# Annusha/LIReC

Hardware: AMD Instinct MI355X
Metric: clips/sec fwd+bwd at 16 tracks×2048-d (higher is better)
Workload: dtype f32 in/out, bf16x3 split-precision MFMA, f32 accumulate

## Files before the change

### lirec_amd/csrc/gemm.hpp

```cpp
#pragma once
#include <hip/hip_runtime.h>
#include <stdint.h>

namespace lirec {

typedef float f32x16 __attribute__((ext_vector_type(16)));
typedef float f32x4 __attribute__((ext_vector_type(4)));

enum { L_NT = 0, L_NN = 1, L_TN = 2 };
enum { EPI_STORE = 0, EPI_DROP_RELU = 1, EPI_TANH_DROP = 2, EPI_RELU_BWD = 3, EPI_TANH_BWD = 4 };

struct GemmProblem {
  const float* A; const float* B; float* C;
  const float* bias;
  const float* rowscale;
  const float* aux;
  float* aux_out;
  float* dbias;
  long lda, ldb, ldc, ldaux;
  int M, N, K;
  int gs, gstride, goff;
  unsigned gs_magic;
  int epi; float beta;
  int dbias_set;
  unsigned seed_lo, seed_hi, site, thresh; float drop_scale; int drop_col_off;
  const unsigned long long* seed_dev;
  int x_bf16;
  int tiles_n, tile_start;
  int ksplit, kchunk, tiles_mn;
  float* slab; float* dbias_slab;
  const int* rowmap; const int* dyn;
  const int* srow;
  const void* A_lo; const void* B_lo;
  unsigned char* xq_out; long ld_xq;
};

struct AdamFuse {
  float* p; const float* g; float* m; float* v;
  float step_size, bc2_sqrt, beta1, beta2, eps, wd, gscale, lr;
  const long long* step_dev;
  int wq16c;
};
struct AdamHyperRow {
  float lr, beta1, beta2, eps, wd, decoupled, pad_[2];
// ... 33 lines not shown
    if constexpr (DECOUPLED) gg = gv[j] * ad.gscale;
    else gg = gv[j] * ad.gscale + ad.wd * pv[j];
    mv[j] = mv[j] + (1.f - ad.beta1) * (gg - mv[j]);
    vv[j] = vv[j] * ad.beta2 + (1.f - ad.beta2) * gg * gg;
    const float denom = sqrtf(vv[j]) / bc2_sqrt + ad.eps;
    if constexpr (DECOUPLED) pv[j] = pv[j] * decay;
    pv[j] = pv[j] - step_size * (mv[j] / denom);
  }
  *reinterpret_cast<f32x4*>(ad.p + off) = pv;
  *reinterpret_cast<f32x4*>(ad.m + off) = mv;
  *reinterpret_cast<f32x4*>(ad.v + off) = vv;
  return pv;
}

#define LIREC_MAX_PROB 8
struct GemmGroup {
  int nprob; int total_tiles; int ablate; int row_tiles;
  const int* nt_bound;
  int nt_bound_val;
  int p3_tm, p3_tn, p3_xm;
  int nt_ct_major;
  int onepass;
  int tier_rows, row_tiles2, first2;
  int pgroup;
  int tm_fast;
  int tiles_per_split, resident_slots, dyn_is_k;
  int dyn_split;
  float slab_cost, reduce_cost;
  GemmProblem p[LIREC_MAX_PROB];
};
struct GemmMeta { int site; int tag; };

inline bool gemm_problem_is_vec(int layout, const GemmProblem& p) {
  const bool a_kc = layout != 2, b_kc = layout == 0;
  const uintptr_t ma = (p.x_bf16 && layout == 0) ? 7 : 15, mb = (p.x_bf16 && layout == 2) ? 7 : 15;
  const bool va = ((p.lda & 3) == 0) && ((reinterpret_cast<uintptr_t>(p.A) & ma) == 0) && (((a_kc ? p.K : p.M) & 3) == 0);
  const bool vb = ((p.ldb & 3) == 0) && ((reinterpret_cast<uintptr_t>(p.B) & mb) == 0) && (((b_kc ? p.K : p.N) & 3) == 0);
  return va && vb;
}

__device__ __forceinline__ void philox4(unsigned c0, unsigned c1, unsigned c2, unsigned c3,
                                        unsigned k0, unsigned k1, unsigned out[4]) {
#pragma unroll 2
// ... 102 lines not shown
}

template <int ST = 64>
__device__ __forceinline__ int xcd_remap(int bid, int nwg) {
  const int full = nwg - nwg % (8 * ST);
  const int xcd = bid & 7;
  if (bid < full) {
    const int seq = bid >> 3;
    return ((seq / ST) * 8 + xcd) * ST + seq % ST;
  }
  const int n = nwg - full, q = n >> 3, r = n & 7;
  const int idx = (bid - full) >> 3;
  return full + (xcd < r ? xcd * (q + 1) : r * (q + 1) + (xcd - r) * q) + idx;
}

__device__ __forceinline__ int effective_ksplit(const GemmGroup& g, const GemmProblem& p, int K) {
  if (p.ksplit <= 1 || !g.dyn_split || !(g.ablate & 64)) return p.ksplit;
  int best = 1;
  float bestc = 3.0e38f;
  for (int ks = 1; ks <= p.ksplit; ++ks) {
    const int nk = ((K + ks - 1) / ks + 31) / 32;
    if (ks > 1 && nk < 8) break;
    const int rounds = (g.tiles_per_split * ks + g.resident_slots - 1) / g.resident_slots;
    const float c = (float)rounds * (float)nk + (ks > 1 ? g.reduce_cost + g.slab_cost * (float)(ks + 1) : 0.f);
    if (c < bestc) { bestc = c; best = ks; }
  }
  return best;
}

__device__ __forceinline__ int launch_tile(const GemmGroup& g) {
  int nwg = gridDim.x;
  if (g.dyn_split && g.dyn_is_k && (g.ablate & 64)) {
    const GemmProblem& p0 = g.p[0];
    const int ks = effective_ksplit(g, p0, dyn_limit(p0, p0.K));
    nwg = g.tiles_per_split * ks;
    if ((int)blockIdx.x >= nwg) return -1;
  }
  return g.pgroup > 0 ? xcd_remap<32>(blockIdx.x, nwg) : xcd_remap<64>(blockIdx.x, nwg);
}

struct TileCoord { int pi, split, m0, n0, tn, k_begin, k_end, M; };
template <int BM, int BN>
__device__ __forceinline__ TileCoord decode_tile(const GemmGroup& g, int tile, bool dyn_is_k) {
  TileCoord c;
  c.pi = 0;
  int tm;
  if (g.pgroup > 0) {
    const int G = g.pgroup, tier1 = g.tier_rows * g.row_tiles;
    const bool t2 = g.row_tiles2 > 0 && tile >= tier1;
    const int first = t2 ? g.first2 : 0, np = t2 ? g.nprob - g.first2 : g.nprob;
    const int rt = t2 ? g.row_tiles2 : g.row_tiles;
    const int rows = t2 ? g.p[first].tiles_mn / g.p[first].tiles_n - g.tier_rows : g.tier_rows;
    const int t = t2 ? tile - tier1 : tile;
    const int tn_each = g.p[first].tiles_n;
    const int blk = t / (G * rt);
    const int within = t - blk * G * rt;
    const int per = min(G, rows - blk * G) * tn_each;
    const int q = within / per, r2 = within - q * per;
    const int rot = (blk * np) / 8 + (t2 ? 1 : 0);
    c.pi = first + (q + rot) % np;
    const int pr = r2 / tn_each;
    c.tn = r2 - pr * tn_each;
    c.split = 0;
    tm = (t2 ? g.tier_rows : 0) + blk * G + pr;
  } else if (g.row_tiles > 0) {
    const int tier1 = g.tier_rows * g.row_tiles;
    if (g.row_tiles2 > 0 && tile >= tier1) {
      const int t2 = tile - tier1;
      const int row2 = t2 / g.row_tiles2;
      const int rem = t2 - row2 * g.row_tiles2 + g.p[g.first2].tile_start;
      c.pi = g.first2;
#pragma unroll
      for (int i = 1; i < LIREC_MAX_PROB; ++i)
        if (i > g.first2 && i < g.nprob && rem >= g.p[i].tile_start) c.pi = i;
      c.tn = rem - g.p[c.pi].tile_start;
      c.split = 0;
      tm = g.tier_rows + row2;
    } else {
      const int tiles_m = g.p[0].tiles_mn / g.p[0].tiles_n;
      int row, rem;
      if (g.tm_fast) {
        const int per_split = tiles_m * g.row_tiles;
        c.split = tile / per_split;
        const int r = tile - c.split * per_split;
        rem = r / tiles_m;
        tm = r - rem * tiles_m;
      } else {
        row = tile / g.row_tiles;
        rem = tile - row * g.row_tiles;
        c.split = row / tiles_m;
        tm = row - c.split * tiles_m;
      }
#pragma unroll
      for (int i = 1; i < LIREC_MAX_PROB; ++i)
        if (i < g.nprob && rem >= g.p[i].tile_start) c.pi = i;
      c.tn = rem - g.p[c.pi].tile_start;
    }
  } else {
#pragma unroll
    for (int i = 1; i < LIREC_MAX_PROB; ++i)
      if (i < g.nprob && tile >= g.p[i].tile_start) c.pi = i;
    int t = tile - g.p[c.pi].tile_start;
    c.split = t / g.p[c.pi].tiles_mn;
    t -= c.split * g.p[c.pi].tiles_mn;
    tm = t / g.p[c.pi].tiles_n;
    c.tn = t - tm * g.p[c.pi].tiles_n;
  }
  const GemmProblem& p = g.p[c.pi];
  c.m0 = tm * BM; c.n0 = c.tn * BN;
  int K = p.K, kchunk = p.kchunk;
  c.M = p.M;
  if (p.dyn) {
    if (dyn_is_k) {
      K = dyn_limit(p, p.K);
      const int ks = effective_ksplit(g, p, K);
      kchunk = ((K + ks - 1) / ks + 31) / 32 * 32;
      if (c.split >= ks) c.M = 0;
    } else {
      c.M = dyn_limit(p, p.M);
    }
  }
  c.k_begin = min(K, c.split * kchunk);
  c.k_end = min(K, c.k_begin + kchunk);
  return c;
}

template <int WM, int WN, int EPI>
__device__ __forceinline__ void gemm_epilogue_kind(const GemmProblem& p, const f32x16 (&acc)[WM][WN], int m0, int n0,
                                                   int wm0, int wn0, int lane, int M, bool have_rid = false, int rid_lane = 0) {
  constexpr bool USES_RND = (EPI == EPI_DROP_RELU || EPI == EPI_TANH_DROP || EPI == EPI_TANH_BWD);
  constexpr bool USES_AUX = (EPI == EPI_RELU_BWD || EPI == EPI_TANH_BWD);
  const int l31 = lane & 31, lh = lane >> 5;
  const int N = p.N;
  const bool drop = USES_RND && p.thresh != 0u;
  unsigned key_lo = p.seed_lo, key_hi = p.seed_hi;
  if (drop) apply_seed_offset(key_lo, key_hi, p.seed_dev);
  const bool mapped = drop && (p.rowmap != nullptr);
  const bool has_beta = p.beta != 0.f, has_rs = p.bias != nullptr && p.rowscale != nullptr;
  float bias_j[WN];
#pragma unroll
  for (int j = 0; j < WN; ++j) {
    const int col = n0 + wn0 + 32 * j + l31;
    bias_j[j] = (p.bias != nullptr && col < N) ? p.bias[col] : 0.f;
  }
  constexpr bool PRE_AUX = USES_AUX && (WM * WN <= 2);
#pragma unroll
  for (int i = 0; i < WM; ++i) {
#pragma unroll
    for (int j = 0; j < WN; ++j) {
      const int col = n0 + wn0 + 32 * j + l31;
      const bool colok = col < N;
      float axp[PRE_AUX ? 16 : 1];
      if constexpr (PRE_AUX) {
#pragma unroll
        for (int q = 0; q < 4; ++q)
#pragma unroll
          for (int jj = 0; jj < 4; ++jj) {
            const int row = m0 + wm0 + 32 * i + 8 * q + 4 * lh + jj;
            const bool okk = colok && row < M;
            axp[4 * q + jj] = p.aux[(long)(okk ? row : m0) * p.ldaux + (okk ? col : n0)];
          }
      }
#pragma unroll
      for (int q = 0; q < 4; ++q) {
        const int row4 = m0 + wm0 + 32 * i + 8 * q + 4 * lh;
        if (row4 >= M) continue;
        bool ok[4];
        float* cptr[4];
        float old[4] = {0.f, 0.f, 0.f, 0.f}, ax[4] = {0.f, 0.f, 0.f, 0.f}, rs[4] = {1.f, 1.f, 1.f, 1.f};
#pragma unroll
        for (int jj = 0; jj < 4; ++jj) {
          ok[jj] = colok && (row4 + jj < M);
          const int r = ok[jj] ? row4 + jj : m0, c = ok[jj] ? col : n0;
          cptr[jj] = p.C + (long)r * p.ldc + c;
          if (has_beta) old[jj] = *cptr[jj];
          if constexpr (PRE_AUX) ax[jj] = axp[4 * q + jj];
          else if constexpr (USES_AUX) ax[jj] = p.aux[(long)r * p.ldaux + c];
          if (has_rs) rs[jj] = p.rowscale[r];
        }
        unsigned w[4] = {0u, 0u, 0u, 0u};
        if (drop) {
          if (!mapped) {
            philox4((unsigned)(p.drop_col_off + col), (unsigned)(row4 >> 2), p.site, 0u, key_lo, key_hi, w);
          } else {
            unsigned rid[4], rnd[4];
#pragma unroll
            for (int jj = 0; jj < 4; ++jj) {
              if (have_rid) rid[jj] = (unsigned)__shfl(rid_lane, 32 * i + 8 * q + 4 * lh + jj, 64);
              else rid[jj] = (unsigned)p.rowmap[row4 + jj < M ? row4 + jj : M - 1];
            }
            unsigned blk = rid[0] >> 2;
            philox4((unsigned)(p.drop_col_off + col), blk, p.site, 0u, key_lo, key_hi, rnd);
#pragma unroll
// ... 26 lines not shown
          }
          if (ok[jj]) *cptr[jj] = v;
        }
        __asm__ volatile("" ::: "memory");
      }
    }
  }
}

__host__ __device__ constexpr bool epi_allowed(int layout, int epi) {
  return epi == EPI_STORE || (layout == L_NT && (epi == EPI_DROP_RELU || epi == EPI_TANH_DROP)) ||
         (layout == L_NN && (epi == EPI_RELU_BWD || epi == EPI_TANH_BWD));
}

template <int WM, int WN, int LAYOUT>
__device__ __forceinline__ void gemm_epilogue(const GemmProblem& p, const f32x16 (&acc)[WM][WN], int m0, int n0,
                                              int wm0, int wn0, int lane, int split, int M_eff, bool have_rid = false, int rid_lane = 0) {
  const int l31 = lane & 31, lh = lane >> 5;
  const int M = M_eff, N = p.N;
  if (p.ksplit > 1) {
    float* slab = p.slab + (long)split * p.M * N;
#pragma unroll
    for (int i = 0; i < WM; ++i)
#pragma unroll
      for (int j = 0; j < WN; ++j) {
        const int col = n0 + wn0 + 32 * j + l31;
#pragma unroll
        for (int r = 0; r < 16; ++r) {
          const int row = m0 + wm0 + 32 * i + (r & 3) + 8 * (r >> 2) + 4 * lh;
          if (row < M && col < N) slab[(long)row * N + col] = acc[i][j][r];
        }
      }
    return;
  }
  if constexpr (LAYOUT == L_NT) {
    if (p.epi == EPI_DROP_RELU) gemm_epilogue_kind<WM, WN, EPI_DROP_RELU>(p, acc, m0, n0, wm0, wn0, lane, M, have_rid, rid_lane);
    else if (p.epi == EPI_TANH_DROP) gemm_epilogue_kind<WM, WN, EPI_TANH_DROP>(p, acc, m0, n0, wm0, wn0, lane, M);
    else gemm_epilogue_kind<WM, WN, EPI_STORE>(p, acc, m0, n0, wm0, wn0, lane, M);
  } else if constexpr (LAYOUT == L_NN) {
    if (p.epi == EPI_RELU_BWD) gemm_epilogue_kind<WM, WN, EPI_RELU_BWD>(p, acc, m0, n0, wm0, wn0, lane, M);
    else if (p.epi == EPI_TANH_BWD) gemm_epilogue_kind<WM, WN, EPI_TANH_BWD>(p, acc, m0, n0, wm0, wn0, lane, M);
    else gemm_epilogue_kind<WM, WN, EPI_STORE>(p, acc, m0, n0, wm0, wn0, lane, M);
  } else {
    gemm_epilogue_kind<WM, WN, EPI_STORE>(p, acc, m0, n0, wm0, wn0, lane, M);
  }
}

static __global__ __launch_bounds__(256) void splitk_reduce_kernel(const GemmGroup g) {
  for (int pi = 0; pi < g.nprob; ++pi) {
    const GemmProblem& p = g.p[pi];
    if (p.ksplit <= 1) continue;
    const int ks = (p.dyn && g.dyn_is_k) ? effective_ksplit(g, p, dyn_limit(p, p.K)) : p.ksplit;
    const long mn = (long)p.M * p.N;
    const long gtid = (long)blockIdx.x * blockDim.x + threadIdx.x, gsz = (long)gridDim.x * blockDim.x;
    const bool vec4 = (p.N % 4 == 0) && (p.ldc % 4 == 0) && ((((size_t)p.C) | ((size_t)p.slab)) % 16 == 0);
    if (p.epi != EPI_STORE) {
      const bool drop = p.thresh != 0u && (p.epi == EPI_DROP_RELU || p.epi == EPI_TANH_DROP || p.epi == EPI_TANH_BWD);
      unsigned key_lo = p.seed_lo, key_hi = p.seed_hi;
      if (drop) apply_seed_offset(key_lo, key_hi, p.seed_dev);
      const long groups = (long)((p.M + 3) >> 2) * p.N;
      for (long e = gtid; e < groups; e += gsz) {
        const int r4 = (int)(e / p.N), col = (int)(e - (long)r4 * p.N), row0 = r4 << 2;
        float v[4] = {0.f, 0.f, 0.f, 0.f};
        for (int sidx = 0; sidx < ks; ++sidx) {
          const float* sl = p.slab + (long)sidx * mn + (long)row0 * p.N + col;
#pragma unroll
          for (int jj = 0; jj < 4; ++jj) if (row0 + jj < p.M) v[jj] += sl[(long)jj * p.N];
// ... 61 lines not shown
        *c = v;
      }
    }
    if (p.dbias && p.dbias_slab) {
      for (int m = blockIdx.x * blockDim.x + threadIdx.x; m < p.M; m += gridDim.x * blockDim.x) {
        float v = 0.f;
        for (int s = 0; s < ks; ++s) v += p.dbias_slab[(long)s * p.M + m];
        p.dbias[m] = p.dbias_set ? v : p.dbias[m] + v;
      }
    }
  }
}

struct ReducePlan { int n; int start[LIREC_MAX_PROB + 1]; int prob[LIREC_MAX_PROB]; };
static __global__ __launch_bounds__(256) void splitk_reduce_flat_kernel(const GemmGroup g, const ReducePlan rp) {
  int k = 0;
  while (k + 1 < rp.n && (int)blockIdx.x >= rp.start[k + 1]) ++k;
  const GemmProblem& p = g.p[rp.prob[k]];
  const int ks = p.ksplit;
  const long mn = (long)p.M * p.N;
  const long e = (long)((int)blockIdx.x - rp.start[k]) * 256 + threadIdx.x;
  const bool vec4 = (p.N % 4 == 0) && (p.ldc % 4 == 0) && ((((size_t)p.C) | ((size_t)p.slab)) % 16 == 0);
  if (vec4) {
    const long mn4 = mn >> 2;
    const int n4 = p.N >> 2;
    if (e < mn4) {
      const int row = (int)(e / n4), col = (int)(e - (long)row * n4) * 4;
      const f32x4* src = (const f32x4*)p.slab + e;
      f32x4* c = (f32x4*)(p.C + (long)row * p.ldc + col);
      f32x4 o = {0.f, 0.f, 0.f, 0.f};
      if (p.beta != 0.f) o = *c;
      f32x4 v = src[0];
      int s = 1;
      for (; s + 3 < ks; s += 4) {
        const f32x4 t0 = src[(long)s * mn4], t1 = src[(long)(s + 1) * mn4], t2 = src[(long)(s + 2) * mn4], t3 = src[(long)(s + 3) * mn4];
#pragma unroll
// ... 37 lines not shown

template <int LAYOUT, int WM, int WN, int TAG, bool VEC>
__global__ __launch_bounds__(256) void gemm_mfma_kernel(const GemmGroup g) {
  constexpr int BM = 64 * WM, BN = 64 * WN, BK = 32;
  constexpr bool A_KC = (LAYOUT != L_TN);
  constexpr bool B_KC = (LAYOUT == L_NT);
  constexpr int PA = A_KC ? BM + 1 : BM + 4;
  constexpr int PB = B_KC ? BN + 1 : BN + 4;
  constexpr int A_TILE = BK * PA, B_TILE = BK * PB;
  constexpr int CA = BM / 32, CB = BN / 32;
  __shared__ __attribute__((aligned(16))) float smem[2 * (A_TILE + B_TILE)];
  float* const As = smem;
  float* const Bs = smem + 2 * A_TILE;

  const int tid = threadIdx.x, lane = tid & 63, wave = tid >> 6;
  const int ltile = launch_tile(g);
  if (ltile < 0) return;
  const TileCoord tc = decode_tile<BM, BN>(g, ltile, LAYOUT == L_TN);
  const GemmProblem& p = g.p[tc.pi];
  const int m0 = tc.m0, n0 = tc.n0, tn = tc.tn;
  const int M = tc.M, N = p.N, K = tc.k_end;
  if (m0 >= M) return;

  const float* a_rowptr[CA];
  const float* b_rowptr[CB];
  bool a_rowok[CA], b_rowok[CB];
  if constexpr (A_KC) {
#pragma unroll
    for (int i = 0; i < CA; ++i) {
      const int m = m0 + (tid >> 3) + 32 * i;
      a_rowok[i] = m < M;
      a_rowptr[i] = p.A + (LAYOUT == L_NT ? phys_row(p, a_rowok[i] ? m : 0) : (long)(a_rowok[i] ? m : 0)) * p.lda;
    }
  }
  if constexpr (B_KC) {
#pragma unroll
    for (int i = 0; i < CB; ++i) {
// ... 120 lines not shown
    }
    if (do_dbias) {
      const float* ac = As + buf * A_TILE + tid;
      if (p.rowscale) {
        const int kbase = kb + kt * BK;
        for (int k = 0; k < BK; ++k) dbias_acc += ac[k * PA] * ((kbase + k < K) ? p.rowscale[kbase + k] : 0.f);
      } else {
#pragma unroll 8
        for (int k = 0; k < BK; ++k) dbias_acc += ac[k * PA];
      }
    }
    if (kt + 1 < nk) store_tiles(buf ^ 1, kb + (kt + 1) * BK);
    __syncthreads();
  }

  gemm_epilogue<WM, WN, LAYOUT>(p, acc, m0, n0, wm0, wn0, lane, tc.split, M);
  if (do_dbias && m0 + tid < M) {
    if (p.ksplit > 1) p.dbias_slab[(long)tc.split * p.M + m0 + tid] = dbias_acc;
    else p.dbias[m0 + tid] = p.dbias_set ? dbias_acc : p.dbias[m0 + tid] + dbias_acc;
  }
}

template <int LAYOUT>
__global__ void gemm_naive_kernel(const GemmProblem p) {
  const int col = blockIdx.x * 16 + (threadIdx.x & 15);
  const int row = blockIdx.y * 16 + (threadIdx.x >> 4);
  const int M = (LAYOUT == L_TN) ? p.M : dyn_limit(p, p.M);
  const int K = (LAYOUT == L_TN) ? dyn_limit(p, p.K) : p.K;
  if (row >= M || col >= p.N) return;
  float acc = 0.f;
  if (LAYOUT == L_NT) {
    const long arow = phys_row(p, row) * p.lda;
    const float* a = p.A + arow;
// ... 28 lines not shown
```

### lirec_amd/csrc/gemm_bf16x3.hpp

```cpp
#pragma once
#include <type_traits>
#include "gemm.hpp"

namespace lirec {

typedef __bf16 bf16x8 __attribute__((ext_vector_type(8)));
typedef __bf16 bf16x4 __attribute__((ext_vector_type(4)));
typedef short s16x4 __attribute__((ext_vector_type(4)));
typedef short s16x8 __attribute__((ext_vector_type(8)));

typedef float f32x2 __attribute__((ext_vector_type(2)));
typedef __bf16 bf16x2 __attribute__((ext_vector_type(2)));
__device__ __forceinline__ void split4(const f32x4 v, uint2& hi, uint2& lo) {
  const f32x2 v01 = {v[0], v[1]}, v23 = {v[2], v[3]};
  const bf16x2 h01 = __builtin_convertvector(v01, bf16x2), h23 = __builtin_convertvector(v23, bf16x2);
  const unsigned w01 = __builtin_bit_cast(unsigned, h01), w23 = __builtin_bit_cast(unsigned, h23);
  const f32x2 f01 = {__builtin_bit_cast(float, w01 << 16), __builtin_bit_cast(float, w01 & 0xffff0000u)};
  const f32x2 f23 = {__builtin_bit_cast(float, w23 << 16), __builtin_bit_cast(float, w23 & 0xffff0000u)};
  const f32x2 r01 = v01 - f01, r23 = v23 - f23;
  const bf16x2 l01 = __builtin_convertvector(r01, bf16x2), l23 = __builtin_convertvector(r23, bf16x2);
  hi = make_uint2(w01, w23);
  lo = make_uint2(__builtin_bit_cast(unsigned, l01), __builtin_bit_cast(unsigned, l23));
}

// ... 55 lines not shown
  constexpr bool A_KC = (LAYOUT != L_TN);
  constexpr bool B_KC = (LAYOUT == L_NT);
  static_assert(!XB || (VEC && LAYOUT != L_NN), "bf16 X: dword-aligned staging, forward or weight-gradient layout");
  constexpr bool AXB = XB && LAYOUT == L_NT, BXB = XB && LAYOUT == L_TN;
  using TA = OperandTile<A_KC, BM>;
  using TB = OperandTile<B_KC, BN>;
  constexpr int BUF = 2 * (TA::BYTES + TB::BYTES);
  constexpr int RP = NTHR / 8;
  constexpr int QA = BM / 4, QB = BN / 4;
  constexpr int KSA = NTHR / QA, KSB = NTHR / QB;
  constexpr int CA = A_KC ? BM / RP : BK / KSA;
  constexpr int CB = B_KC ? BN / RP : BK / KSB;
  __shared__ __attribute__((aligned(16))) unsigned char smem[2 * BUF];

  const int tid = threadIdx.x, lane = tid & 63, wave = tid >> 6;
  const int ltile = launch_tile(g);
  if (ltile < 0) return;
  const TileCoord tc = decode_tile<BM, BN>(g, ltile, LAYOUT == L_TN);
  const GemmProblem& p = g.p[tc.pi];
  const int m0 = tc.m0, n0 = tc.n0;
  const int M = tc.M, N = p.N, K = tc.k_end, kb = tc.k_begin;
  if (m0 >= M) return;
  const bool interior = (m0 + BM <= M) && (n0 + BN <= N) && (((K - kb) & (BK - 1)) == 0);

  const float* a_rowptr[A_KC ? CA : 1];
  const float* b_rowptr[B_KC ? CB : 1];
  bool a_rowok[A_KC ? CA : 1], b_rowok[B_KC ? CB : 1];
  if constexpr (A_KC) {
#pragma unroll
    for (int i = 0; i < CA; ++i) {
      const int m = m0 + (tid >> 3) + RP * i;
      a_rowok[i] = m < M;
      const long arow = (LAYOUT == L_NT ? phys_row(p, a_rowok[i] ? m : 0) : (long)(a_rowok[i] ? m : 0)) * p.lda;
      a_rowptr[i] = AXB ? reinterpret_cast<const float*>(reinterpret_cast<const char*>(p.A) + 2 * arow) : p.A + arow;
    }
  }
  if constexpr (B_KC) {
// ... 127 lines not shown
          *reinterpret_cast<uint2*>(b_hi + off) = h;
          *reinterpret_cast<uint2*>(b_lo + off) = l;
        }
      }
    }
  };
  f32x16 acc[WM][WN];
#pragma unroll
  for (int i = 0; i < WM; ++i)
#pragma unroll
    for (int j = 0; j < WN; ++j)
#pragma unroll
      for (int r = 0; r < 16; ++r) acc[i][j][r] = 0.f;

  const int wm0 = (wave / WAVES_N) * 32 * WM, wn0 = (wave % WAVES_N) * 32 * WN;
  const int l31 = lane & 31, lh = lane >> 5;
  const int kc_swz = (lane >> 2) & 3;
  const int kc_s0 = 16 * (lh ^ (kc_swz & 1)) + 32 * (kc_swz >> 1);
  const int a_frag = A_KC ? (wm0 + l31) * TA::PITCH + kc_s0
                          : (8 * lh + ((lane & 15) >> 2)) * TA::PITCH + 2 * (wm0 + 16 * ((lane >> 4) & 1) + 4 * (lane & 3));
  const int b_frag = B_KC ? (wn0 + l31) * TB::PITCH + kc_s0
                          : (8 * lh + ((lane & 15) >> 2)) * TB::PITCH + 2 * (wn0 + 16 * ((lane >> 4) & 1) + 4 * (lane & 3));

  auto frag_a = [&](const unsigned char* img, int i, int s) -> bf16x8 {
    if constexpr (A_KC) {
      return *reinterpret_cast<const bf16x8*>(img + (a_frag ^ (32 * s)) + 32 * TA::PITCH * i);
    } else {
      const unsigned char* q = img + a_frag + 64 * i + 16 * s * TA::PITCH;
      const s16x4 x = lds_tr16(q), y = lds_tr16(q + 4 * TA::PITCH);
      const s16x8 v = {x[0], x[1], x[2], x[3], y[0], y[1], y[2], y[3]};
// ... 74 lines not shown
      ++kt;
    }
    ktile(kt & 1, 0, 0, std::false_type{}, std::false_type{}, edge_tag, one_tag);
    __syncthreads();
  };
  constexpr bool ONE_OK = !(LAYOUT == L_TN && TAG == 0 && (CFG == 1 || CFG == 2 || CFG == 4));
  bool one = false;
  if constexpr (ONE_OK) one = g.onepass != 0;
  if (g.ablate & 4) {  }
  else if (one) {
    if constexpr (ONE_OK) { if (interior) mainloop(std::false_type{}, std::true_type{}); else mainloop(std::true_type{}, std::true_type{}); }
  }
  else if (interior) mainloop(std::false_type{}, std::false_type{});
  else mainloop(std::true_type{}, std::false_type{});

  gemm_epilogue<WM, WN, LAYOUT>(p, acc, m0, n0, wm0, wn0, lane, tc.split, M);

  if constexpr (LAYOUT == L_TN) {
    if (do_dbias) {
      float* red = reinterpret_cast<float*>(smem);
      __syncthreads();
#pragma unroll
      for (int c = 0; c < 4; ++c) red[tid * 4 + c] = dbias_acc[c];
      __syncthreads();
      if (tid < QA) {
        float v[4] = {0.f, 0.f, 0.f, 0.f};
        for (int r = 0; r < KSA; ++r)
#pragma unroll
          for (int c = 0; c < 4; ++c) v[c] += red[(tid + QA * r) * 4 + c];
#pragma unroll
        for (int c = 0; c < 4; ++c) {
          const int m = m0 + 4 * tid + c;
          if (m < M) {
            if (p.ksplit > 1) p.dbias_slab[(long)tc.split * p.M + m] = v[c];
            else p.dbias[m] = p.dbias_set ? v[c] : p.dbias[m] + v[c];
          }
        }
      }
    }
  }
}

}
```

### lirec_amd/csrc/lirec_hip.hip

```cpp
#include <hip/hip_runtime.h>
#include <math.h>
#include <stdlib.h>
#include <string.h>
#include <new>

#include "lirec_hip.h"
#include "gemm.hpp"
#include "gemm_launch.hpp"
#include "kernels.hpp"
#include "gemm_dx.hpp"

using namespace lirec;

thread_local lirec::CmdList* lirec::t_rec = nullptr;
bool lirec::g_dry = false;
struct lirec_cmdlist { lirec::CmdList list; };

struct lirec_ctx {
  int gemm_mode = 0;
  int ablate = 0;
  int force_cfg = -1;
  float* scratch = nullptr;
  long scratch_floats = 0;
};
// ... 111 lines not shown

static inline GemmProblem make_problem() {
  GemmProblem q;
  memset(&q, 0, sizeof(q));
  q.drop_scale = 1.f;
  return q;
}

static int plan_tiles_v(GemmGroup& g, int bm, int bn, const int* ks_want, bool& any_split) {
  int start = 0;
  long scratch_off = 0;
  any_split = false;
  for (int i = 0; i < g.nprob; ++i) {
    GemmProblem& p = g.p[i];
    const int tm = (p.M + bm - 1) / bm, tn = (p.N + bn - 1) / bn;
    p.tiles_n = tn > 0 ? tn : 1;
    p.tiles_mn = tm * tn;
    p.tile_start = start;
    int ks = ks_want[i];
    const int max_ks = p.K / 256 > 0 ? p.K / 256 : 1;
    if (ks > max_ks) ks = max_ks;
    if (ks > 32) ks = 32;
    if (ks < 1) ks = 1;
    int kchunk = ((p.K + ks - 1) / ks + 31) / 32 * 32;
    ks = (p.K + kchunk - 1) / kchunk;
    const long need = (long)ks * p.M * p.N + (p.dbias ? (long)ks * p.M : 0);
    if (ks > 1 && scratch_off + need <= g_scratch_floats) {
      p.ksplit = ks; p.kchunk = kchunk;
      p.slab = g_scratch + scratch_off;
      p.dbias_slab = p.dbias ? p.slab + (long)ks * p.M * p.N : nullptr;
      scratch_off += need;
      any_split = true;
    } else {
      p.ksplit = 1; p.kchunk = (p.K + 31) / 32 * 32; p.slab = nullptr; p.dbias_slab = nullptr;
    }
    start += (p.M > 0 && p.N > 0) ? tm * tn * p.ksplit : 0;
  }
  g.total_tiles = start;
  g.row_tiles = 0; g.tier_rows = 0; g.row_tiles2 = 0; g.first2 = 0; g.pgroup = 0; g.tm_fast = 0;
  {
    long tiles = 0, mn_total = 0;
    for (int i = 0; i < g.nprob; ++i) { tiles += g.p[i].tiles_mn; mn_total += (long)g.p[i].M * g.p[i].N; }
    const double tk = (bm * bn >= 256 * 256) ? 2.8 : (bm * bn >= 256 * 128 ? 1.6 : 1.2);
    g.tiles_per_split = (int)tiles;
    g.resident_slots = (bm * bn > 128 * 128) ? 256 : 512;
    g.slab_cost = (float)((double)mn_total * 4.0 / 4.0e6 / tk);
    g.reduce_cost = (float)(6.0 / tk);
  }
  if (start == 0) return 0;
  if (g.nprob > 1) {
    auto tiles_m = [&](int i) { return g.p[i].tiles_mn / g.p[i].tiles_n; };
    bool same = true, unsplit = g.p[0].ksplit == 1;
    for (int i = 1; i < g.nprob; ++i) {
      same = same && tiles_m(i) == tiles_m(0) && g.p[i].ksplit == g.p[0].ksplit;
      unsplit = unsplit && g.p[i].ksplit == 1;
    }
    int first2 = 0;
    bool two = !same && unsplit;
    if (two) {
      while (first2 < g.nprob && tiles_m(first2) == tiles_m(0)) ++first2;
      two = first2 < g.nprob && tiles_m(first2) > tiles_m(0);
      for (int i = first2; two && i < g.nprob; ++i) two = tiles_m(i) == tiles_m(first2);
    }
    if (same || two) {
      int off = 0;
      for (int i = 0; i < g.nprob; ++i) { g.p[i].tile_start = off; off += g.p[i].tiles_n; }
      g.row_tiles = off;
      g.tier_rows = tiles_m(0);
      if (two) { g.first2 = first2; g.row_tiles2 = off - g.p[first2].tile_start; }
      bool eq = unsplit && !(g_ablate & 256);
      for (int i = 1; i < g.nprob; ++i) eq = eq && g.p[i].tiles_n == g.p[0].tiles_n;
      const int tn = g.p[0].tiles_n;
      if (eq && tn <= 16 && 32 % tn == 0 && g.tier_rows >= 32 / tn) g.pgroup = 32 / tn;
    }
  }
  {
    bool ok = g.p[0].ksplit > 1 && g.p[0].dyn != nullptr && (g.nprob == 1 || (g.row_tiles > 0 && g.row_tiles2 == 0));
    for (int i = 1; ok && i < g.nprob; ++i) ok = g.p[i].ksplit == g.p[0].ksplit && g.p[i].dyn == g.p[0].dyn && g.p[i].K == g.p[0].K;
    g.dyn_split = ok ? 1 : 0;
  }
  g.tm_fast = (g.dyn_is_k && g.row_tiles > 0 && g.row_tiles2 == 0 && !(g_ablate & 512)) ? 1 : 0;
  return start;
}
static void launch_splitk_reduce(const GemmGroup& g, hipStream_t s) {
  ReducePlan rp;
  memset(&rp, 0, sizeof(rp));
  bool plain = !(g_ablate & (64 | 128 | 4096));
  int blocks = 0;
  for (int i = 0; i < g.nprob; ++i) {
    const GemmProblem& p = g.p[i];
    if (p.ksplit <= 1) continue;
    plain = plain && p.epi == EPI_STORE && !(p.dyn && g.dyn_split && (g_ablate & 64));
    const bool vec4 = (p.N % 4 == 0) && (p.ldc % 4 == 0) && ((((size_t)p.C) | ((size_t)p.slab)) % 16 == 0);
    long items = vec4 ? ((long)p.M * p.N) >> 2 : (long)p.M * p.N;
    if (p.dbias && p.dbias_slab && items < p.M) items = p.M;
    rp.prob[rp.n] = i;
    rp.start[rp.n++] = blocks;
    blocks += (int)((items + 255) / 256);
  }
  rp.start[rp.n] = blocks;
  if (plain && rp.n > 0 && blocks > 0) lirec::launch(splitk_reduce_flat_kernel, dim3((unsigned)blocks), dim3(256), 0, s, g, rp);
  else lirec::launch(splitk_reduce_kernel, dim3(1024), dim3(256), 0, s, g);
}

static int plan_tiles(GemmGroup& g, int bm, int bn, int ksplit_want, bool& any_split) {
  int ks[LIREC_MAX_PROB];
// ... 10 lines not shown
  double flops = 0.0;
  for (int i = 0; i < g.nprob; ++i) flops += 2.0 * g.p[i].M * (double)g.p[i].N * g.p[i].K;
  const int pi = prof_start(meta.site, s);
  const int rc = launch_layout_<LAYOUT>(g, meta, s);
  prof_stop(pi, s, flops, 0.0);
  return rc;
}

template <int LAYOUT>
static int launch_layout_(GemmGroup& g, GemmMeta meta, hipStream_t s) {
  for (int i = 0; i < g.nprob; ++i)
    if (!epi_allowed(LAYOUT, g.p[i].epi)) return LIREC_EINVAL;
  if (g_gemm_mode == 1) {
    for (int i = 0; i < g.nprob; ++i) {
      GemmProblem& p = g.p[i];
      p.ksplit = 1;
      if (p.M <= 0 || p.N <= 0) continue;
      dim3 grid((p.N + 15) / 16, (p.M + 15) / 16);
      if (LAYOUT == L_NT) launch_naive_L0(grid, s, p);
      else if (LAYOUT == L_NN) launch_naive_L1(grid, s, p);
      else launch_naive_L2(grid, s, p);
      LIREC_CHECK_LAUNCH();
    }
    return LIREC_OK;
  }
  long t256 = 0, t128 = 0, t64 = 0, mn_total = 0;
  bool splittable = g_scratch != nullptr && !t_no_split, wide = true, wide256 = true, deep = true, any_epi = false;
  for (int i = 0; i < g.nprob; ++i) {
    const GemmProblem& p = g.p[i];
    t256 += (long)((p.M + 255) / 256) * ((p.N + 255) / 256);
    t128 += (long)((p.M + 127) / 128) * ((p.N + 127) / 128);
// ... 2394 lines not shown
```

Before: 82050.

## Move per-problem tile metadata into vectorized group header for scalar-register decode

Per-problem tile bookkeeping (tile_start, tiles_n, tiles_mn, ksplit, kchunk, dyn pointer) moves out of each GemmProblem into packed vector fields of a new GemmHead. The tile locator can then load them with a few wide scalar loads and pick the problem with selects instead of dynamic indexing into the kernel-argument array, and small-tile kernels copy the chosen problem struct into registers. Epilogue bias, rowscale and seed loads are gathered into an EpiPre prefetch that single-wave-tile kernels issue before the main loop, with rowscale broadcast via shuffles. Split detection now checks slab != nullptr. This adds register pressure and changes how the naive path handles ksplit.

Result: slower. 80700 (-1.6%).

```diff
diff --git a/lirec_amd/csrc/gemm.hpp b/lirec_amd/csrc/gemm.hpp
--- a/lirec_amd/csrc/gemm.hpp
+++ b/lirec_amd/csrc/gemm.hpp
@@ -26,8 +26,6 @@
   unsigned seed_lo, seed_hi, site, thresh; float drop_scale; int drop_col_off;
   const unsigned long long* seed_dev;
   int x_bf16;
-  int tiles_n, tile_start;
-  int ksplit, kchunk, tiles_mn;
   float* slab; float* dbias_slab;
   const int* rowmap; const int* dyn;
   const int* srow;
@@ -91,19 +89,26 @@
 }
 
 #define LIREC_MAX_PROB 8
-struct GemmGroup {
+typedef int WordsPerProb __attribute__((ext_vector_type(LIREC_MAX_PROB), aligned(16)));
+typedef unsigned long long AddrPerProb __attribute__((ext_vector_type(LIREC_MAX_PROB), aligned(16)));
+typedef const __attribute__((address_space(4))) int* DynPtr;
+struct GemmHead {
   int nprob; int total_tiles; int ablate; int row_tiles;
+  int tier_rows, row_tiles2, first2;
+  int pgroup;
+  int tm_fast;
+  int dyn_split;
+  int dyn_is_k, tiles_per_split, resident_slots;
+  float slab_cost, reduce_cost;
+  int onepass;
+  WordsPerProb tile_start, tiles_n, tiles_mn, ksplit, kchunk;
+  AddrPerProb dyn;
   const int* nt_bound;
   int nt_bound_val;
   int p3_tm, p3_tn, p3_xm;
   int nt_ct_major;
-  int onepass;
-  int tier_rows, row_tiles2, first2;
-  int pgroup;
-  int tm_fast;
-  int tiles_per_split, resident_slots, dyn_is_k;
-  int dyn_split;
-  float slab_cost, reduce_cost;
+};
+struct GemmGroup : GemmHead {
   GemmProblem p[LIREC_MAX_PROB];
 };
 struct GemmMeta { int site; int tag; };
@@ -236,11 +241,11 @@
   return full + (xcd < r ? xcd * (q + 1) : r * (q + 1) + (xcd - r) * q) + idx;
 }
 
-__device__ __forceinline__ int effective_ksplit(const GemmGroup& g, const GemmProblem& p, int K) {
-  if (p.ksplit <= 1 || !g.dyn_split || !(g.ablate & 64)) return p.ksplit;
+__device__ __forceinline__ int effective_ksplit(const GemmHead& g, int ksplit, int K) {
+  if (ksplit <= 1 || !g.dyn_split || !(g.ablate & 64)) return ksplit;
   int best = 1;
   float bestc = 3.0e38f;
-  for (int ks = 1; ks <= p.ksplit; ++ks) {
+  for (int ks = 1; ks <= ksplit; ++ks) {
     const int nk = ((K + ks - 1) / ks + 31) / 32;
     if (ks > 1 && nk < 8) break;
     const int rounds = (g.tiles_per_split * ks + g.resident_slots - 1) / g.resident_slots;
@@ -250,31 +255,49 @@
   return best;
 }
 
-__device__ __forceinline__ int launch_tile(const GemmGroup& g) {
-  int nwg = gridDim.x;
-  if (g.dyn_split && g.dyn_is_k && (g.ablate & 64)) {
-    const GemmProblem& p0 = g.p[0];
-    const int ks = effective_ksplit(g, p0, dyn_limit(p0, p0.K));
-    nwg = g.tiles_per_split * ks;
+__device__ __forceinline__ int launch_tile(const GemmHead& h, const GemmGroup& g) {
+  int nwg = h.total_tiles;
+  if (h.dyn_split && h.dyn_is_k && (h.ablate & 64)) {
+    const int K0 = g.p[0].K, d = h.dyn[0] ? *(DynPtr)h.dyn[0] : K0;
+    const int ks = effective_ksplit(h, h.ksplit[0], d < K0 ? d : K0);
+    nwg = h.tiles_per_split * ks;
     if ((int)blockIdx.x >= nwg) return -1;
   }
-  return g.pgroup > 0 ? xcd_remap<32>(blockIdx.x, nwg) : xcd_remap<64>(blockIdx.x, nwg);
+  return h.pgroup > 0 ? xcd_remap<32>(blockIdx.x, nwg) : xcd_remap<64>(blockIdx.x, nwg);
+}
+
+struct TileWords { int tile_start, tiles_n, tiles_mn, ksplit, kchunk; DynPtr dyn; };
+__device__ __forceinline__ TileWords tile_words(const GemmHead& h, int pi) {
+  return TileWords{h.tile_start[pi], h.tiles_n[pi], h.tiles_mn[pi], h.ksplit[pi], h.kchunk[pi], (DynPtr)h.dyn[pi]};
+}
+__device__ __forceinline__ int last_start_le(const GemmHead& h, int lo, int x) {
+  int pi = lo;
+#pragma unroll
+  for (int i = 1; i < LIREC_MAX_PROB; ++i)
+    if (i > lo && i < h.nprob && x >= h.tile_start[i]) pi = i;
+  return pi;
 }
 
 struct TileCoord { int pi, split, m0, n0, tn, k_begin, k_end, M; };
-template <int BM, int BN>
-__device__ __forceinline__ TileCoord decode_tile(const GemmGroup& g, int tile, bool dyn_is_k) {
-  TileCoord c;
+template <int BM, int BN, bool COPY>
+__device__ __forceinline__ bool locate_tile(const GemmGroup& g, bool dyn_is_k, TileCoord& c, GemmProblem& pcopy) {
+  const GemmHead h = g;
+  __asm__ volatile("" :: "s"(h.nprob), "s"(h.tile_start), "s"(h.tiles_n), "s"(h.tiles_mn), "s"(h.ksplit), "s"(h.kchunk), "s"(h.dyn));
+  const int tile = launch_tile(h, g);
+  if (tile < 0) return false;
   c.pi = 0;
+  c.split = 0;
   int tm;
-  if (g.pgroup > 0) {
-    const int G = g.pgroup, tier1 = g.tier_rows * g.row_tiles;
-    const bool t2 = g.row_tiles2 > 0 && tile >= tier1;
-    const int first = t2 ? g.first2 : 0, np = t2 ? g.nprob - g.first2 : g.nprob;
-    const int rt = t2 ? g.row_tiles2 : g.row_tiles;
-    const int rows = t2 ? g.p[first].tiles_mn / g.p[first].tiles_n - g.tier_rows : g.tier_rows;
+  TileWords w;
+  if (h.pgroup > 0) {
+    const int G = h.pgroup, tier1 = h.tier_rows * h.row_tiles;
+    const bool t2 = h.row_tiles2 > 0 && tile >= tier1;
+    const int first = t2 ? h.first2 : 0, np = t2 ? h.nprob - h.first2 : h.nprob;
+    const int rt = t2 ? h.row_tiles2 : h.row_tiles;
+    const TileWords wf = tile_words(h, first);
+    const int rows = t2 ? wf.tiles_mn / wf.tiles_n - h.tier_rows : h.tier_rows;
     const int t = t2 ? tile - tier1 : tile;
-    const int tn_each = g.p[first].tiles_n;
+    const int tn_each = wf.tiles_n;
     const int blk = t / (G * rt);
     const int within = t - blk * G * rt;
     const int per = min(G, rows - blk * G) * tn_each;
@@ -283,88 +306,100 @@
     c.pi = first + (q + rot) % np;
     const int pr = r2 / tn_each;
     c.tn = r2 - pr * tn_each;
-    c.split = 0;
-    tm = (t2 ? g.tier_rows : 0) + blk * G + pr;
-  } else if (g.row_tiles > 0) {
-    const int tier1 = g.tier_rows * g.row_tiles;
-    if (g.row_tiles2 > 0 && tile >= tier1) {
+    tm = (t2 ? h.tier_rows : 0) + blk * G + pr;
+    w = tile_words(h, c.pi);
+  } else if (h.row_tiles > 0) {
+    const int tier1 = h.tier_rows * h.row_tiles;
+    if (h.row_tiles2 > 0 && tile >= tier1) {
       const int t2 = tile - tier1;
-      const int row2 = t2 / g.row_tiles2;
-      const int rem = t2 - row2 * g.row_tiles2 + g.p[g.first2].tile_start;
-      c.pi = g.first2;
-#pragma unroll
-      for (int i = 1; i < LIREC_MAX_PROB; ++i)
-        if (i > g.first2 && i < g.nprob && rem >= g.p[i].tile_start) c.pi = i;
-      c.tn = rem - g.p[c.pi].tile_start;
-      c.split = 0;
-      tm = g.tier_rows + row2;
+      const int row2 = t2 / h.row_tiles2;
+      const int rem = t2 - row2 * h.row_tiles2 + tile_words(h, h.first2).tile_start;
+      c.pi = last_start_le(h, h.first2, rem);
+      w = tile_words(h, c.pi);
+      c.tn = rem - w.tile_start;
+      tm = h.tier_rows + row2;
     } else {
-      const int tiles_m = g.p[0].tiles_mn / g.p[0].tiles_n;
+      const int tiles_m = h.tiles_mn[0] / h.tiles_n[0];
       int row, rem;
-      if (g.tm_fast) {
-        const int per_split = tiles_m * g.row_tiles;
+      if (h.tm_fast) {
+        const int per_split = tiles_m * h.row_tiles;
         c.split = tile / per_split;
         const int r = tile - c.split * per_split;
         rem = r / tiles_m;
         tm = r - rem * tiles_m;
       } else {
-        row = tile / g.row_tiles;
-        rem = tile - row * g.row_tiles;
+        row = tile / h.row_tiles;
+        rem = tile - row * h.row_tiles;
         c.split = row / tiles_m;
         tm = row - c.split * tiles_m;
       }
-#pragma unroll
-      for (int i = 1; i < LIREC_MAX_PROB; ++i)
-        if (i < g.nprob && rem >= g.p[i].tile_start) c.pi = i;
-      c.tn = rem - g.p[c.pi].tile_start;
+      c.pi = last_start_le(h, 0, rem);
+      w = tile_words(h, c.pi);
+      c.tn = rem - w.tile_start;
     }
   } else {
-#pragma unroll
-    for (int i = 1; i < LIREC_MAX_PROB; ++i)
-      if (i < g.nprob && tile >= g.p[i].tile_start) c.pi = i;
-    int t = tile - g.p[c.pi].tile_start;
-    c.split = t / g.p[c.pi].tiles_mn;
-    t -= c.split * g.p[c.pi].tiles_mn;
-    tm = t / g.p[c.pi].tiles_n;
-    c.tn = t - tm * g.p[c.pi].tiles_n;
-  }
-  const GemmProblem& p = g.p[c.pi];
+    c.pi = last_start_le(h, 0, tile);
+    w = tile_words(h, c.pi);
+    int t = tile - w.tile_start;
+    c.split = t / w.tiles_mn;
+    t -= c.split * w.tiles_mn;
+    tm = t / w.tiles_n;
+    c.tn = t - tm * w.tiles_n;
+  }
+  if constexpr (COPY) pcopy = g.p[c.pi];
+  const GemmProblem& p = COPY ? static_cast<const GemmProblem&>(pcopy) : g.p[c.pi];
+  int d = 0;
+  if (w.dyn) d = *w.dyn;
   c.m0 = tm * BM; c.n0 = c.tn * BN;
-  int K = p.K, kchunk = p.kchunk;
+  int K = p.K, kchunk = w.kchunk;
   c.M = p.M;
-  if (p.dyn) {
+  if (w.dyn) {
     if (dyn_is_k) {
-      K = dyn_limit(p, p.K);
-      const int ks = effective_ksplit(g, p, K);
+      K = d < p.K ? d : p.K;
+      const int ks = effective_ksplit(h, w.ksplit, K);
       kchunk = ((K + ks - 1) / ks + 31) / 32 * 32;
       if (c.split >= ks) c.M = 0;
     } else {
-      c.M = dyn_limit(p, p.M);
+      c.M = d < p.M ? d : p.M;
     }
   }
   c.k_begin = min(K, c.split * kchunk);
   c.k_end = min(K, c.k_begin + kchunk);
-  return c;
-}
-
+  return c.m0 < c.M;
+}
+
+template <int WN> struct EpiPre { float bias_j[WN]; unsigned key_lo, key_hi; float rs_lane; };
+template <int WM, int WN>
+__device__ __forceinline__ EpiPre<WN> epi_fetch(const GemmProblem& p, int m0, int n0, int wm0, int wn0, int lane, int M) {
+  EpiPre<WN> e;
+  e.rs_lane = 1.f;
+  if constexpr (WM <= 2) {
+    if (p.bias != nullptr && p.rowscale != nullptr) {
+      const int row = m0 + wm0 + lane;
+      e.rs_lane = p.rowscale[(lane < 32 * WM && row < M) ? row : m0];
+    }
+  }
+#pragma unroll
+  for (int j = 0; j < WN; ++j) {
+    const int col = n0 + wn0 + 32 * j + (lane & 31);
+    e.bias_j[j] = (p.bias != nullptr && col < p.N) ? p.bias[col] : 0.f;
+  }
+  e.key_lo = p.seed_lo; e.key_hi = p.seed_hi;
+  if (epi_uses_dropout(p)) apply_seed_offset(e.key_lo, e.key_hi, p.seed_dev);
+  return e;
+}
 template <int WM, int WN, int EPI>
-__device__ __forceinline__ void gemm_epilogue_kind(const GemmProblem& p, const f32x16 (&acc)[WM][WN], int m0, int n0,
+__device__ __forceinline__ void gemm_epilogue_kind(const GemmProblem& p, const EpiPre<WN>& pre, const f32x16 (&acc)[WM][WN], int m0, int n0,
                                                    int wm0, int wn0, int lane, int M, bool have_rid = false, int rid_lane = 0) {
   constexpr bool USES_RND = (EPI == EPI_DROP_RELU || EPI == EPI_TANH_DROP || EPI == EPI_TANH_BWD);
   constexpr bool USES_AUX = (EPI == EPI_RELU_BWD || EPI == EPI_TANH_BWD);
   const int l31 = lane & 31, lh = lane >> 5;
   const int N = p.N;
   const bool drop = USES_RND && p.thresh != 0u;
-  unsigned key_lo = p.seed_lo, key_hi = p.seed_hi;
-  if (drop) apply_seed_offset(key_lo, key_hi, p.seed_dev);
+  const unsigned key_lo = pre.key_lo, key_hi = pre.key_hi;
   const bool mapped = drop && (p.rowmap != nullptr);
   const bool has_beta = p.beta != 0.f, has_rs = p.bias != nullptr && p.rowscale != nullptr;
-  float bias_j[WN];
-#pragma unroll
-  for (int j = 0; j < WN; ++j) {
-    const int col = n0 + wn0 + 32 * j + l31;
-    bias_j[j] = (p.bias != nullptr && col < N) ? p.bias[col] : 0.f;
-  }
+  const float (&bias_j)[WN] = pre.bias_j;
   constexpr bool PRE_AUX = USES_AUX && (WM * WN <= 2);
 #pragma unroll
   for (int i = 0; i < WM; ++i) {
@@ -386,10 +421,17 @@
 #pragma unroll
       for (int q = 0; q < 4; ++q) {
         const int row4 = m0 + wm0 + 32 * i + 8 * q + 4 * lh;
+        float rs[4] = {1.f, 1.f, 1.f, 1.f};
+        if constexpr (WM <= 2) {
+          if (has_rs) {
+#pragma unroll
+            for (int jj = 0; jj < 4; ++jj) rs[jj] = __shfl(pre.rs_lane, 32 * i + 8 * q + 4 * lh + jj, 64);
+          }
+        }
         if (row4 >= M) continue;
         bool ok[4];
         float* cptr[4];
-        float old[4] = {0.f, 0.f, 0.f, 0.f}, ax[4] = {0.f, 0.f, 0.f, 0.f}, rs[4] = {1.f, 1.f, 1.f, 1.f};
+        float old[4] = {0.f, 0.f, 0.f, 0.f}, ax[4] = {0.f, 0.f, 0.f, 0.f};
 #pragma unroll
         for (int jj = 0; jj < 4; ++jj) {
           ok[jj] = colok && (row4 + jj < M);
@@ -398,7 +440,7 @@
           if (has_beta) old[jj] = *cptr[jj];
           if constexpr (PRE_AUX) ax[jj] = axp[4 * q + jj];
           else if constexpr (USES_AUX) ax[jj] = p.aux[(long)r * p.ldaux + c];
-          if (has_rs) rs[jj] = p.rowscale[r];
+          if constexpr (WM > 2) { if (has_rs) rs[jj] = p.rowscale[r]; }
         }
         unsigned w[4] = {0u, 0u, 0u, 0u};
         if (drop) {
@@ -455,11 +497,11 @@
 }
 
 template <int WM, int WN, int LAYOUT>
-__device__ __forceinline__ void gemm_epilogue(const GemmProblem& p, const f32x16 (&acc)[WM][WN], int m0, int n0,
+__device__ __forceinline__ void gemm_epilogue(const GemmProblem& p, const EpiPre<WN>& pre, const f32x16 (&acc)[WM][WN], int m0, int n0,
                                               int wm0, int wn0, int lane, int split, int M_eff, bool have_rid = false, int rid_lane = 0) {
   const int l31 = lane & 31, lh = lane >> 5;
   const int M = M_eff, N = p.N;
-  if (p.ksplit > 1) {
+  if (p.slab != nullptr) {
     float* slab = p.slab + (long)split * p.M * N;
 #pragma unroll
     for (int i = 0; i < WM; ++i)
@@ -475,23 +517,23 @@
     return;
   }
   if constexpr (LAYOUT == L_NT) {
-    if (p.epi == EPI_DROP_RELU) gemm_epilogue_kind<WM, WN, EPI_DROP_RELU>(p, acc, m0, n0, wm0, wn0, lane, M, have_rid, rid_lane);
-    else if (p.epi == EPI_TANH_DROP) gemm_epilogue_kind<WM, WN, EPI_TANH_DROP>(p, acc, m0, n0, wm0, wn0, lane, M);
-    else gemm_epilogue_kind<WM, WN, EPI_STORE>(p, acc, m0, n0, wm0, wn0, lane, M);
+    if (p.epi == EPI_DROP_RELU) gemm_epilogue_kind<WM, WN, EPI_DROP_RELU>(p, pre, acc, m0, n0, wm0, wn0, lane, M, have_rid, rid_lane);
+    else if (p.epi == EPI_TANH_DROP) gemm_epilogue_kind<WM, WN, EPI_TANH_DROP>(p, pre, acc, m0, n0, wm0, wn0, lane, M);
+    else gemm_epilogue_kind<WM, WN, EPI_STORE>(p, pre, acc, m0, n0, wm0, wn0, lane, M);
   } else if constexpr (LAYOUT == L_NN) {
-    if (p.epi == EPI_RELU_BWD) gemm_epilogue_kind<WM, WN, EPI_RELU_BWD>(p, acc, m0, n0, wm0, wn0, lane, M);
-    else if (p.epi == EPI_TANH_BWD) gemm_epilogue_kind<WM, WN, EPI_TANH_BWD>(p, acc, m0, n0, wm0, wn0, lane, M);
-    else gemm_epilogue_kind<WM, WN, EPI_STORE>(p, acc, m0, n0, wm0, wn0, lane, M);
+    if (p.epi == EPI_RELU_BWD) gemm_epilogue_kind<WM, WN, EPI_RELU_BWD>(p, pre, acc, m0, n0, wm0, wn0, lane, M);
+    else if (p.epi == EPI_TANH_BWD) gemm_epilogue_kind<WM, WN, EPI_TANH_BWD>(p, pre, acc, m0, n0, wm0, wn0, lane, M);
+    else gemm_epilogue_kind<WM, WN, EPI_STORE>(p, pre, acc, m0, n0, wm0, wn0, lane, M);
   } else {
-    gemm_epilogue_kind<WM, WN, EPI_STORE>(p, acc, m0, n0, wm0, wn0, lane, M);
+    gemm_epilogue_kind<WM, WN, EPI_STORE>(p, pre, acc, m0, n0, wm0, wn0, lane, M);
   }
 }
 
 static __global__ __launch_bounds__(256) void splitk_reduce_kernel(const GemmGroup g) {
   for (int pi = 0; pi < g.nprob; ++pi) {
     const GemmProblem& p = g.p[pi];
-    if (p.ksplit <= 1) continue;
-    const int ks = (p.dyn && g.dyn_is_k) ? effective_ksplit(g, p, dyn_limit(p, p.K)) : p.ksplit;
+    if (g.ksplit[pi] <= 1) continue;
+    const int ks = (p.dyn && g.dyn_is_k) ? effective_ksplit(g, g.ksplit[pi], dyn_limit(p, p.K)) : g.ksplit[pi];
     const long mn = (long)p.M * p.N;
     const long gtid = (long)blockIdx.x * blockDim.x + threadIdx.x, gsz = (long)gridDim.x * blockDim.x;
     const bool vec4 = (p.N % 4 == 0) && (p.ldc % 4 == 0) && ((((size_t)p.C) | ((size_t)p.slab)) % 16 == 0);
@@ -583,12 +625,16 @@
 
 struct ReducePlan { int n; int start[LIREC_MAX_PROB + 1]; int prob[LIREC_MAX_PROB]; };
 static __global__ __launch_bounds__(256) void splitk_reduce_flat_kernel(const GemmGroup g, const ReducePlan rp) {
-  int k = 0;
-  while (k + 1 < rp.n && (int)blockIdx.x >= rp.start[k + 1]) ++k;
-  const GemmProblem& p = g.p[rp.prob[k]];
-  const int ks = p.ksplit;
+  const ReducePlan r = rp;
+  int first = r.start[0], pi = r.prob[0];
+#pragma unroll
+  for (int i = 1; i < LIREC_MAX_PROB; ++i)
+    if (i < r.n && (int)blockIdx.x >= r.start[i]) { first = r.start[i]; pi = r.prob[i]; }
+  const WordsPerProb ksplit = g.ksplit;
+  const int ks = ksplit[pi];
+  const GemmProblem p = g.p[pi];
   const long mn = (long)p.M * p.N;
-  const long e = (long)((int)blockIdx.x - rp.start[k]) * 256 + threadIdx.x;
+  const long e = (long)((int)blockIdx.x - first) * 256 + threadIdx.x;
   const bool vec4 = (p.N % 4 == 0) && (p.ldc % 4 == 0) && ((((size_t)p.C) | ((size_t)p.slab)) % 16 == 0);
   if (vec4) {
     const long mn4 = mn >> 2;
@@ -656,13 +702,13 @@
   float* const Bs = smem + 2 * A_TILE;
 
   const int tid = threadIdx.x, lane = tid & 63, wave = tid >> 6;
-  const int ltile = launch_tile(g);
-  if (ltile < 0) return;
-  const TileCoord tc = decode_tile<BM, BN>(g, ltile, LAYOUT == L_TN);
-  const GemmProblem& p = g.p[tc.pi];
+  constexpr bool COPY = WM * WN <= 2;
+  TileCoord tc;
+  GemmProblem pcopy;
+  if (!locate_tile<BM, BN, COPY>(g, LAYOUT == L_TN, tc, pcopy)) return;
+  const GemmProblem& p = COPY ? static_cast<const GemmProblem&>(pcopy) : g.p[tc.pi];
   const int m0 = tc.m0, n0 = tc.n0, tn = tc.tn;
   const int M = tc.M, N = p.N, K = tc.k_end;
-  if (m0 >= M) return;
 
   const float* a_rowptr[CA];
   const float* b_rowptr[CB];
@@ -813,9 +859,9 @@
     __syncthreads();
   }
 
-  gemm_epilogue<WM, WN, LAYOUT>(p, acc, m0, n0, wm0, wn0, lane, tc.split, M);
+  gemm_epilogue<WM, WN, LAYOUT>(p, epi_fetch<WM, WN>(p, m0, n0, wm0, wn0, lane, M), acc, m0, n0, wm0, wn0, lane, tc.split, M);
   if (do_dbias && m0 + tid < M) {
-    if (p.ksplit > 1) p.dbias_slab[(long)tc.split * p.M + m0 + tid] = dbias_acc;
+    if (p.slab != nullptr) p.dbias_slab[(long)tc.split * p.M + m0 + tid] = dbias_acc;
     else p.dbias[m0 + tid] = p.dbias_set ? dbias_acc : p.dbias[m0 + tid] + dbias_acc;
   }
 }
diff --git a/lirec_amd/csrc/gemm_bf16x3.hpp b/lirec_amd/csrc/gemm_bf16x3.hpp
--- a/lirec_amd/csrc/gemm_bf16x3.hpp
+++ b/lirec_amd/csrc/gemm_bf16x3.hpp
@@ -93,13 +93,13 @@
   __shared__ __attribute__((aligned(16))) unsigned char smem[2 * BUF];
 
   const int tid = threadIdx.x, lane = tid & 63, wave = tid >> 6;
-  const int ltile = launch_tile(g);
-  if (ltile < 0) return;
-  const TileCoord tc = decode_tile<BM, BN>(g, ltile, LAYOUT == L_TN);
-  const GemmProblem& p = g.p[tc.pi];
+  constexpr bool EPI_EARLY = WM * WN <= 2;
+  TileCoord tc;
+  GemmProblem pcopy;
+  if (!locate_tile<BM, BN, EPI_EARLY>(g, LAYOUT == L_TN, tc, pcopy)) return;
+  const GemmProblem& p = EPI_EARLY ? static_cast<const GemmProblem&>(pcopy) : g.p[tc.pi];
   const int m0 = tc.m0, n0 = tc.n0;
   const int M = tc.M, N = p.N, K = tc.k_end, kb = tc.k_begin;
-  if (m0 >= M) return;
   const bool interior = (m0 + BM <= M) && (n0 + BN <= N) && (((K - kb) & (BK - 1)) == 0);
 
   const float* a_rowptr[A_KC ? CA : 1];
@@ -257,6 +257,9 @@
       for (int r = 0; r < 16; ++r) acc[i][j][r] = 0.f;
 
   const int wm0 = (wave / WAVES_N) * 32 * WM, wn0 = (wave % WAVES_N) * 32 * WN;
+  constexpr bool FETCH_EARLY = WM * WN == 1;
+  EpiPre<WN> pre;
+  if constexpr (FETCH_EARLY) pre = epi_fetch<WM, WN>(p, m0, n0, wm0, wn0, lane, M);
   const int l31 = lane & 31, lh = lane >> 5;
   const int kc_swz = (lane >> 2) & 3;
   const int kc_s0 = 16 * (lh ^ (kc_swz & 1)) + 32 * (kc_swz >> 1);
@@ -361,7 +364,8 @@
   else if (interior) mainloop(std::false_type{}, std::false_type{});
   else mainloop(std::true_type{}, std::false_type{});
 
-  gemm_epilogue<WM, WN, LAYOUT>(p, acc, m0, n0, wm0, wn0, lane, tc.split, M);
+  if constexpr (!FETCH_EARLY) pre = epi_fetch<WM, WN>(p, m0, n0, wm0, wn0, lane, M);
+  gemm_epilogue<WM, WN, LAYOUT>(p, pre, acc, m0, n0, wm0, wn0, lane, tc.split, M);
 
   if constexpr (LAYOUT == L_TN) {
     if (do_dbias) {
@@ -379,7 +383,7 @@
         for (int c = 0; c < 4; ++c) {
           const int m = m0 + 4 * tid + c;
           if (m < M) {
-            if (p.ksplit > 1) p.dbias_slab[(long)tc.split * p.M + m] = v[c];
+            if (p.slab != nullptr) p.dbias_slab[(long)tc.split * p.M + m] = v[c];
             else p.dbias[m] = p.dbias_set ? v[c] : p.dbias[m] + v[c];
           }
         }
diff --git a/lirec_amd/csrc/lirec_hip.hip b/lirec_amd/csrc/lirec_hip.hip
--- a/lirec_amd/csrc/lirec_hip.hip
+++ b/lirec_amd/csrc/lirec_hip.hip
@@ -149,9 +149,10 @@
   for (int i = 0; i < g.nprob; ++i) {
     GemmProblem& p = g.p[i];
     const int tm = (p.M + bm - 1) / bm, tn = (p.N + bn - 1) / bn;
-    p.tiles_n = tn > 0 ? tn : 1;
-    p.tiles_mn = tm * tn;
-    p.tile_start = start;
+    g.tiles_n[i] = tn > 0 ? tn : 1;
+    g.tiles_mn[i] = tm * tn;
+    g.tile_start[i] = start;
+    g.dyn[i] = (unsigned long long)reinterpret_cast<uintptr_t>(p.dyn);
     int ks = ks_want[i];
     const int max_ks = p.K / 256 > 0 ? p.K / 256 : 1;
     if (ks > max_ks) ks = max_ks;
@@ -161,21 +162,21 @@
     ks = (p.K + kchunk - 1) / kchunk;
     const long need = (long)ks * p.M * p.N + (p.dbias ? (long)ks * p.M : 0);
     if (ks > 1 && scratch_off + need <= g_scratch_floats) {
-      p.ksplit = ks; p.kchunk = kchunk;
+      g.ksplit[i] = ks; g.kchunk[i] = kchunk;
       p.slab = g_scratch + scratch_off;
       p.dbias_slab = p.dbias ? p.slab + (long)ks * p.M * p.N : nullptr;
       scratch_off += need;
       any_split = true;
     } else {
-      p.ksplit = 1; p.kchunk = (p.K + 31) / 32 * 32; p.slab = nullptr; p.dbias_slab = nullptr;
-    }
-    start += (p.M > 0 && p.N > 0) ? tm * tn * p.ksplit : 0;
+      g.ksplit[i] = 1; g.kchunk[i] = (p.K + 31) / 32 * 32; p.slab = nullptr; p.dbias_slab = nullptr;
+    }
+    start += (p.M > 0 && p.N > 0) ? tm * tn * g.ksplit[i] : 0;
   }
   g.total_tiles = start;
   g.row_tiles = 0; g.tier_rows = 0; g.row_tiles2 = 0; g.first2 = 0; g.pgroup = 0; g.tm_fast = 0;
   {
     long tiles = 0, mn_total = 0;
-    for (int i = 0; i < g.nprob; ++i) { tiles += g.p[i].tiles_mn; mn_total += (long)g.p[i].M * g.p[i].N; }
+    for (int i = 0; i < g.nprob; ++i) { tiles += g.tiles_mn[i]; mn_total += (long)g.p[i].M * g.p[i].N; }
     const double tk = (bm * bn >= 256 * 256) ? 2.8 : (bm * bn >= 256 * 128 ? 1.6 : 1.2);
     g.tiles_per_split = (int)tiles;
     g.resident_slots = (bm * bn > 128 * 128) ? 256 : 512;
@@ -184,11 +185,11 @@
   }
   if (start == 0) return 0;
   if (g.nprob > 1) {
-    auto tiles_m = [&](int i) { return g.p[i].tiles_mn / g.p[i].tiles_n; };
-    bool same = true, unsplit = g.p[0].ksplit == 1;
+    auto tiles_m = [&](int i) { return g.tiles_mn[i] / g.tiles_n[i]; };
+    bool same = true, unsplit = g.ksplit[0] == 1;
     for (int i = 1; i < g.nprob; ++i) {
-      same = same && tiles_m(i) == tiles_m(0) && g.p[i].ksplit == g.p[0].ksplit;
-      unsplit = unsplit && g.p[i].ksplit == 1;
+      same = same && tiles_m(i) == tiles_m(0) && g.ksplit[i] == g.ksplit[0];
+      unsplit = unsplit && g.ksplit[i] == 1;
     }
     int first2 = 0;
     bool two = !same && unsplit;
@@ -199,19 +200,19 @@
     }
     if (same || two) {
       int off = 0;
-      for (int i = 0; i < g.nprob; ++i) { g.p[i].tile_start = off; off += g.p[i].tiles_n; }
+      for (int i = 0; i < g.nprob; ++i) { g.tile_start[i] = off; off += g.tiles_n[i]; }
       g.row_tiles = off;
       g.tier_rows = tiles_m(0);
-      if (two) { g.first2 = first2; g.row_tiles2 = off - g.p[first2].tile_start; }
+      if (two) { g.first2 = first2; g.row_tiles2 = off - g.tile_start[first2]; }
       bool eq = unsplit && !(g_ablate & 256);
-      for (int i = 1; i < g.nprob; ++i) eq = eq && g.p[i].tiles_n == g.p[0].tiles_n;
-      const int tn = g.p[0].tiles_n;
+      for (int i = 1; i < g.nprob; ++i) eq = eq && g.tiles_n[i] == g.tiles_n[0];
+      const int tn = g.tiles_n[0];
       if (eq && tn <= 16 && 32 % tn == 0 && g.tier_rows >= 32 / tn) g.pgroup = 32 / tn;
     }
   }
   {
-    bool ok = g.p[0].ksplit > 1 && g.p[0].dyn != nullptr && (g.nprob == 1 || (g.row_tiles > 0 && g.row_tiles2 == 0));
-    for (int i = 1; ok && i < g.nprob; ++i) ok = g.p[i].ksplit == g.p[0].ksplit && g.p[i].dyn == g.p[0].dyn && g.p[i].K == g.p[0].K;
+    bool ok = g.ksplit[0] > 1 && g.p[0].dyn != nullptr && (g.nprob == 1 || (g.row_tiles > 0 && g.row_tiles2 == 0));
+    for (int i = 1; ok && i < g.nprob; ++i) ok = g.ksplit[i] == g.ksplit[0] && g.p[i].dyn == g.p[0].dyn && g.p[i].K == g.p[0].K;
     g.dyn_split = ok ? 1 : 0;
   }
   g.tm_fast = (g.dyn_is_k && g.row_tiles > 0 && g.row_tiles2 == 0 && !(g_ablate & 512)) ? 1 : 0;
@@ -224,7 +225,7 @@
   int blocks = 0;
   for (int i = 0; i < g.nprob; ++i) {
     const GemmProblem& p = g.p[i];
-    if (p.ksplit <= 1) continue;
+    if (g.ksplit[i] <= 1) continue;
     plain = plain && p.epi == EPI_STORE && !(p.dyn && g.dyn_split && (g_ablate & 64));
     const bool vec4 = (p.N % 4 == 0) && (p.ldc % 4 == 0) && ((((size_t)p.C) | ((size_t)p.slab)) % 16 == 0);
     long items = vec4 ? ((long)p.M * p.N) >> 2 : (long)p.M * p.N;
@@ -265,7 +266,6 @@
   if (g_gemm_mode == 1) {
     for (int i = 0; i < g.nprob; ++i) {
       GemmProblem& p = g.p[i];
-      p.ksplit = 1;
       if (p.M <= 0 || p.N <= 0) continue;
       dim3 grid((p.N + 15) / 16, (p.M + 15) / 16);
       if (LAYOUT == L_NT) launch_naive_L0(grid, s, p);
```
